# Plonky3/Plonky3-recursion

Measured on AMD Instinct MI355X. Metric: prove_next_layer ms + Poseidon2 perms/s, KoalaBear 2^20-row circuit, 1/8 GPU, lower is better.
Workload: dtype u32 Montgomery (31-bit prime field, degree-4 extension); Poseidon2 hashing as exact integers in f64; 1 GPU; prove_next_layer (verifier-circuit run on the device + prove_all_tables) of the synthetic koala-bear 2^20-row recursion layer: tables const/public/alu/poseidon2/recompose, FRI blowup 4, arity<=4, 54 queries, 15-bit PoW; circuit inputs + NextLayerPrepCache resident in HBM; field=koala-bear, log_height=20, independent_proofs=1, proof_bytes=612900, parallelism=1 independent proofs, one per GPU, no data-path collective

## Files before the change

### plonky3_recursion_amd/csrc/circuit_impl.hip.h

```cpp

#include "circuit_host.h"

namespace {

template <class PP, int D = 4>
__device__ __forceinline__ typename CircuitExt<PP, D>::type w_load(const uint32_t* __restrict__ w, uint32_t id) {
  typename CircuitExt<PP, D>::type e;
  if constexpr (D == 4) {
    const uint4 v = *reinterpret_cast<const uint4*>(w + (size_t)id * 4);
    e.c[0] = Fp<PP>::raw(v.x); e.c[1] = Fp<PP>::raw(v.y); e.c[2] = Fp<PP>::raw(v.z); e.c[3] = Fp<PP>::raw(v.w);
  } else {
#pragma unroll
    for (int k = 0; k < D; ++k) e.c[k] = Fp<PP>::raw(w[(size_t)id * D + k]);
  }
  return e;
}
template <class PP, int D = 4>
__device__ __forceinline__ void w_store(uint32_t* __restrict__ w, uint32_t id, const typename CircuitExt<PP, D>::type& e) {
  if constexpr (D == 4) {
    *reinterpret_cast<uint4*>(w + (size_t)id * 4) = make_uint4(e.c[0].v, e.c[1].v, e.c[2].v, e.c[3].v);
  } else {
#pragma unroll
    for (int k = 0; k < D; ++k) w[(size_t)id * D + k] = e.c[k].v;
  }
// ... 714 lines not shown
  atomicMin(&slot[v & 0x7FFFFFFFu], (uint32_t)k);
}
__global__ void __launch_bounds__(kBlock)
k_pd_check(const uint32_t* __restrict__ ids, size_t n, const uint32_t* __restrict__ row_of_id, size_t n_ids,
           const uint32_t* __restrict__ slot, uint32_t* __restrict__ err) {
  const size_t k = (size_t)blockIdx.x * kBlock + threadIdx.x;
  if (k >= n) return;
  const uint32_t id = ids[k];
  uint32_t code = 0;
  if (id >= n_ids || row_of_id[id] == kNoW) code = 1;
  else if (slot[row_of_id[id] & 0x7FFFFFFFu] != k) code = 2;
  else if (!(row_of_id[id] >> 31)) code = 3;
  if (code) atomicMin(err, ((uint32_t)k << 2) | code);
}

template <class PP>
std::unique_ptr<p3r_dinputs> circuit_inputs_upload(p3r_ctx* ctx, const p3r_circuit* C, const p3r_circuit_inputs* in) {
  if (C->n_public_rows && !in->public_values) fail(P3R_EINVAL, "PublicInputLengthMismatch: public_values is NULL");
  if (C->n_private_rows && !in->private_values) fail(P3R_EINVAL, "PrivateInputLengthMismatch: private_values is NULL");
  const size_t n_p2 = C->counts.n_p2, n_pd = in->n_private_data;
  if (n_pd && (!in->private_data_op_ids || !in->private_data_siblings)) fail(P3R_EINVAL, "private data arrays are NULL");
  auto D = std::make_unique<p3r_dinputs>();
  D->pub = upload_mont<PP>(ctx, in->public_values, C->n_public_rows * ctx->cfg.ext_degree, "public_values");
  D->priv = upload_mont<PP>(ctx, in->private_values, C->n_private_rows * ctx->cfg.ext_degree, "private_values");
  auto private_data = [&](size_t n_pd, const uint32_t* ids_host, const uint32_t* sib_host, size_t per_op, size_t n_rows,
                          const DevBuf& row_of_id, const DevBuf& other_row_of_id, DevBuf& sib, DevBuf& slot, const char* what) {
    sib = upload_mont<PP>(ctx, sib_host, n_pd * per_op, what);
    slot.alloc(std::max<size_t>(n_rows, 1));
    P3R_HIP(fill_async(ctx->stream, slot.p, 0xFF, std::max<size_t>(n_rows, 1) * 4));
    if (!n_pd) return;
    if (!row_of_id.p)
      fail(P3R_EINVAL, "NonPrimitiveOpIdOutOfRange { op_id: %u, max_ops: %zu } (%s)", ids_host[0], C->n_op_ids, what);
    DevBuf ids(n_pd), err(1);
    P3R_HIP(hipMemcpyAsync(ids.p, ids_host, n_pd * 4, hipMemcpyHostToDevice, ctx->stream));
    P3R_HIP(fill_async(ctx->stream, err.p, 0xFF, 4));
    hipLaunchKernelGGL(k_pd_claim, dim3(blocks_for(n_pd)), dim3(kBlock), 0, ctx->stream, ids.p, n_pd, row_of_id.p, C->n_op_ids, slot.p);
    hipLaunchKernelGGL(k_pd_check, dim3(blocks_for(n_pd)), dim3(kBlock), 0, ctx->stream, ids.p, n_pd, row_of_id.p, C->n_op_ids, slot.p, err.p);
    uint32_t e = 0;
    P3R_HIP(copy_sync(ctx->stream, &e, err.p, 4, hipMemcpyDeviceToHost));
    if (e != 0xFFFFFFFFu) {
      const uint32_t id = ids_host[e >> 2];
      switch (e & 3) {
        case 1: {
          uint32_t other = kNoW;
          if (other_row_of_id.p && id < C->n_op_ids) P3R_HIP(copy_sync(ctx->stream, &other, other_row_of_id.p + id, 4, hipMemcpyDeviceToHost));
          if (other != kNoW)
            fail(P3R_EINVAL, "IncorrectNonPrimitiveOpPrivateData: NonPrimitiveOpId(%u) is a permutation of the other width (%s)", id, what);
          fail(P3R_EINVAL, "NonPrimitiveOpIdOutOfRange { op_id: %u, max_ops: %zu }", id, C->n_op_ids);
        }
        case 2: fail(P3R_EINVAL, "IncorrectNonPrimitiveOpPrivateData: private data already set for NonPrimitiveOpId(%u)", id);
        default: fail(P3R_EINVAL, "IncorrectNonPrimitiveOpPrivateData: private data provided for non-Merkle operation NonPrimitiveOpId(%u)", id);
      }
    }
  };
  private_data(n_pd, in->private_data_op_ids, in->private_data_siblings, 8, n_p2, C->d_row_of_op_id, C->d_roww_of_op_id, D->sib, D->slot,
               "private_data_siblings");
  const size_t n_pdw = in->n_private_data_w32;
  if (n_pdw && (!in->private_data_w32_op_ids || !in->private_data_w32_siblings)) fail(P3R_EINVAL, "width-32 private data arrays are NULL");
  private_data(n_pdw, in->private_data_w32_op_ids, in->private_data_w32_siblings, 24, C->counts.n_p2w, C->d_roww_of_op_id, C->d_row_of_op_id,
               D->sib_w, D->slot_w, "private_data_w32_siblings");
  return D;
}

inline void run_raise_error(uint32_t e) {
  if (e != 0xFFFFFFFFu) {
    const uint32_t idx = e >> 3;
    if (idx == 0x1FFFFFFFu) fail(P3R_EINVAL, "WitnessConflict while applying witness_rewrite");
    fail(P3R_EINVAL, "%s at op %u", run_error_text(e & 7), idx);
  }
}

template <class PP>
std::unique_ptr<p3r_dtraces> circuit_run(p3r_ctx* ctx, const p3r_circuit* C, const p3r_dinputs* in,
                                         uint32_t* deferred_err = nullptr) {
  const RunSchedule& S = C->sched;
  const p3r_layer* L = C->layer.get();
  if (!S.deferred_error.empty()) fail(P3R_EINVAL, "%s", S.deferred_error.c_str());
  const size_t n_p2 = C->counts.n_p2;
// ... 79 lines not shown
    }
    dispatch_ext_degree<PP>((int)ext_d, [&](auto dc) {
    constexpr int DD = decltype(dc)::value;
    for (const auto& seg : S.segments) {
      if (seg.narrow) {
        hipLaunchKernelGGL((k_run_levels_narrow<PP, DD>), dim3(1), dim3(kNarrowBlock), 0, ctx->stream, A,
                           C->d_chunk_bounds.p + seg.chunk_begin, seg.n_chunks);
        continue;
      }
      const uint32_t l = seg.l0;
      const uint32_t nl = S.light_off[l + 1] - S.light_off[l], np = S.p2seg_off[l + 1] - S.p2seg_off[l];
      const uint32_t lb = (nl + kBlock - 1) / kBlock, pb = (np * 16 + kBlock - 1) / kBlock;
      const uint32_t nc = S.chain_off[l + 1] - S.chain_off[l], n_long = S.chain_long[l];
      const RunOp* steps = reinterpret_cast<const RunOp*>(C->d_chain_ops.p);
      const RunSchedule::ChainSeg* segs = reinterpret_cast<const RunSchedule::ChainSeg*>(C->d_chains.p) + S.chain_off[l];
      const uint32_t n_short = nc - n_long, cb = (n_short + kBlock / 64 - 1) / (kBlock / 64);
      const uint32_t npw = has_w32 ? S.p2wseg_off[l + 1] - S.p2wseg_off[l] : 0u, pwb = (npw * 32 + kBlock - 1) / kBlock;
      if (lb + pb + cb + pwb)
        hipLaunchKernelGGL((k_run_level<PP, DD>), dim3(pb + cb + lb + pwb), dim3(kBlock), 0, ctx->stream, A, S.p2seg_off[l], np, pb,
                           steps, segs + n_long, n_short, cb, S.light_off[l], nl, has_w32 ? S.p2wseg_off[l] : 0u, npw, pwb);
      if (n_long)
        hipLaunchKernelGGL((k_run_chains_block<PP, DD>), dim3(n_long), dim3(kLongChainBlock), 0, ctx->stream, A, steps, segs);
    }
    if (C->n_rewrite)
      hipLaunchKernelGGL((k_run_rewrite<PP, DD>), dim3(blocks_for(C->n_rewrite)), dim3(kBlock), 0, ctx->stream,
                         C->d_rewrite.p, C->n_rewrite, w.p, err.p);
    });
    if (cn.n_public)
      hipLaunchKernelGGL(k_run_gather<PP>, dim3(blocks_for(cn.n_public * ext_d)), dim3(kBlock), 0, ctx->stream,
                         C->d_public_out.p, cn.n_public, w.p, T->public_values.p, ext_d);
    P3R_HIP(hipGetLastError());
  }
  if (deferred_err) {
    P3R_HIP(hipMemcpyAsync(deferred_err, err.p, 4, hipMemcpyDeviceToHost, ctx->stream));
  } else {
    uint32_t e = 0;
    P3R_HIP(copy_sync(ctx->stream, &e, err.p, 4, hipMemcpyDeviceToHost));
    run_raise_error(e);
  }
  return T;
}

template <class PP>
void dtraces_get(p3r_ctx* ctx, const p3r_layer* L, const p3r_dtraces* t, uint32_t which, uint32_t* out, size_t out_len) {
  const auto& c = L->counts;
  auto plain_at = [&](const uint32_t* src, size_t n) {
    if (out_len != n) fail(P3R_EBUFFER, "array holds %zu values, caller asked for %zu", n, out_len);
    if (!n) return;
    DevBuf tmp(n);
    P3R_HIP(hipMemcpyAsync(tmp.p, src, n * 4, hipMemcpyDeviceToDevice, ctx->stream));
    hipLaunchKernelGGL(k_convert_inplace<PP>, dim3(blocks_for(n)), dim3(kBlock), 0, ctx->stream, tmp.p, n, 0);
    P3R_HIP(copy_sync(ctx->stream, out, tmp.p, n * 4, hipMemcpyDeviceToHost));
  };
  switch (which) {
    case P3R_TRACES_CONST_VALUES: plain_at(t->const_values.p, c.n_const * ctx->cfg.ext_degree); break;
    case P3R_TRACES_PUBLIC_VALUES: plain_at(t->public_values.p, c.n_public * ctx->cfg.ext_degree); break;
    case P3R_TRACES_ALU_VALUES: plain_at(t->alu_values.p, c.n_alu * 4 * ctx->cfg.ext_degree); break;
    case P3R_TRACES_RECOMPOSE_VALUES: plain_at(t->recompose_values.p, c.n_recompose * ctx->cfg.ext_degree); break;
    case P3R_TRACES_RECOMPOSE_COEFF_VALUES:
      plain_at(t->recompose_values.p + c.n_recompose * ctx->cfg.ext_degree, c.n_recompose_coeff * ctx->cfg.ext_degree);
      break;
    case P3R_TRACES_P2_INPUT_VALUES: {
      if (out_len != c.n_p2 * 16) fail(P3R_EBUFFER, "array holds %zu values, caller asked for %zu", c.n_p2 * 16, out_len);
      if (!c.n_p2) break;
      std::vector<uint32_t> full(t->p2->n * 16);
      download<PP>(ctx, t->p2->inputs.get(), full.data());
      std::copy(full.begin(), full.begin() + c.n_p2 * 16, out);
      break;
    }
    case P3R_TRACES_P2_FLAGS: {
// ... 45 lines not shown
```

### plonky3_recursion_amd/csrc/context.h

```cpp
#pragma once
#include <hip/hip_runtime.h>

#include <algorithm>
#include <array>
#include <atomic>
#include <cstdarg>
#include <cstdio>
#include <cstring>
#include <exception>
#include <functional>
#include <map>
#include <memory>
#include <chrono>
#include <mutex>
#include <stdexcept>
#include <string>
#include <thread>
#include <tuple>
#include <vector>

#include "../../include/p3r.h"
#include "error.h"
#include "field.h"
#include "poseidon2.h"
#include "proof_layout.h"
#include "mmcs4.h"

namespace p3r {

template <class Fn>
inline void host_parallel_for(size_t n, size_t min_chunk, Fn fn) {
  const size_t hw = std::max<size_t>(std::thread::hardware_concurrency(), 1);
  const size_t chunks = std::min<size_t>(std::min<size_t>(hw, 16), (n + min_chunk - 1) / std::max<size_t>(min_chunk, 1));
  if (chunks <= 1) { fn((size_t)0, n); return; }
  std::vector<std::exception_ptr> err(chunks);
  std::vector<std::thread> th;
  auto run = [&](size_t c) {
    try { fn(n * c / chunks, n * (c + 1) / chunks); } catch (...) { err[c] = std::current_exception(); }
  };
  for (size_t c = 1; c < chunks; ++c) th.emplace_back(run, c);
  run(0);
  for (auto& t : th) t.join();
  for (auto& e : err) if (e) std::rethrow_exception(e);
}

#define P3R_HIP(expr)                                                                   \
  do {                                                                                  \
    hipError_t e_ = (expr);                                                             \
    if (e_ != hipSuccess)                                                               \
      ::p3r::fail(e_ == hipErrorOutOfMemory ? P3R_ENOMEM : P3R_EHIP, "%s failed: %s",   \
                  #expr, hipGetErrorString(e_));                                        \
  } while (0)

struct DevPool;
struct PoolRegistry {
  std::mutex mu;
// ... 129 lines not shown
}
template <class T>
static __global__ void __launch_bounds__(256) k_copy_small(uint8_t* __restrict__ dst, const uint8_t* __restrict__ src, size_t n) {
  const size_t tid = (size_t)blockIdx.x * 256 + threadIdx.x, nt = (size_t)gridDim.x * 256;
  const size_t nq = n / sizeof(T);
  T* d = reinterpret_cast<T*>(dst);
  const T* q = reinterpret_cast<const T*>(src);
  for (size_t i = tid; i < nq; i += nt) d[i] = q[i];
  const size_t done = nq * sizeof(T);
  if (tid < n - done) dst[done + tid] = src[done + tid];
}
inline hipError_t fill_async(hipStream_t s, void* p, int byte, size_t bytes) {
  if (bytes == 0) return hipSuccess;
  host_mark("launch: fill");
  const uint32_t b = (uint32_t)byte & 0xFFu, pattern = b * 0x01010101u;
  const size_t blocks = std::min<size_t>((bytes / 16 + 255) / 256 + 1, 4096);
  hipLaunchKernelGGL(k_fill_bytes, dim3((unsigned)blocks), dim3(256), 0, s, static_cast<uint8_t*>(p), pattern, bytes);
  return hipGetLastError();
}
inline hipError_t copy_async_kernel(hipStream_t s, void* dst, const void* src, size_t bytes) {
  if (bytes == 0) return hipSuccess;
  host_mark("launch: copy");
  const uintptr_t both = reinterpret_cast<uintptr_t>(dst) | reinterpret_cast<uintptr_t>(src);
  const size_t w = (both & 15) == 0 ? 16 : (both & 3) == 0 ? 4 : 1;
  const size_t blocks = std::min<size_t>((bytes / w + 255) / 256 + 1, 4096);
  uint8_t* d = static_cast<uint8_t*>(dst);
  const uint8_t* q = static_cast<const uint8_t*>(src);
  if (w == 16) hipLaunchKernelGGL(k_copy_small<uint4>, dim3((unsigned)blocks), dim3(256), 0, s, d, q, bytes);
  else if (w == 4) hipLaunchKernelGGL(k_copy_small<uint32_t>, dim3((unsigned)blocks), dim3(256), 0, s, d, q, bytes);
  else hipLaunchKernelGGL(k_copy_small<uint8_t>, dim3((unsigned)blocks), dim3(256), 0, s, d, q, bytes);
  return hipGetLastError();
}

struct HostStage {
  static constexpr size_t kBytes = size_t(4) << 20;
  char* base = nullptr;
  char* base_dev = nullptr;
  size_t off = 0;
  HostStage() = default;
  HostStage(const HostStage&) = delete;
  HostStage& operator=(const HostStage&) = delete;
  ~HostStage() {
    if (base) (void)hipHostFree(base);
  }
  static constexpr size_t kWordBytes = 64;
  hipError_t ensure() {
    if (base) return hipSuccess;
    off = kWordBytes;
    hipError_t e = hipHostMalloc(reinterpret_cast<void**>(&base), kBytes, hipHostMallocMapped | hipHostMallocCoherent);
    if (e != hipSuccess) return e;
    return hipHostGetDevicePointer(reinterpret_cast<void**>(&base_dev), base, 0);
  }
  hipError_t words(uint32_t** out) {
    hipError_t e = ensure();
    *out = reinterpret_cast<uint32_t*>(base);
    return e;
  }
  hipError_t upload(hipStream_t s, void* dst, const void* src, size_t bytes) {
    if (bytes == 0) return hipSuccess;
    if (bytes > kBytes / 4) return copy_sync(s, dst, src, bytes, hipMemcpyHostToDevice);
    {
      hipError_t e = ensure();
      if (e != hipSuccess) return e;
    }
    const size_t need = (bytes + 63) & ~size_t(63);
    if (off + need > kBytes) {
      hipError_t e = hipStreamSynchronize(s);
      if (e != hipSuccess) return e;
      off = kWordBytes;
    }
    std::memcpy(base + off, src, bytes);
    hipError_t e = copy_async_kernel(s, dst, base_dev + off, bytes);
    off += need;
    return e;
  }
};

struct HostLanding {
  char* base = nullptr;
  size_t cap = 0;
  HostLanding() = default;
  HostLanding(const HostLanding&) = delete;
  HostLanding& operator=(const HostLanding&) = delete;
  ~HostLanding() {
    if (base) (void)hipHostFree(base);
  }
  hipError_t fetch(hipStream_t s, const void* dev, size_t bytes, const uint32_t** out) {
    if (bytes > cap) {
      if (base) (void)hipHostFree(base);
      base = nullptr;
      cap = 0;
      const size_t want = std::max(bytes * 2, size_t(1) << 20);
      hipError_t e = hipHostMalloc(reinterpret_cast<void**>(&base), want, hipHostMallocDefault);
      if (e != hipSuccess) return e;
      cap = want;
    }
    *out = reinterpret_cast<const uint32_t*>(base);
    if (bytes == 0) return hipStreamSynchronize(s);
    return copy_sync(s, base, dev, bytes, hipMemcpyDeviceToHost);
  }
};

static __global__ void __launch_bounds__(256) k_post_small(uint32_t* host_dst, const uint32_t* __restrict__ src, uint32_t n,
                                                    uint32_t* flag, uint32_t seq) {
  for (uint32_t i = threadIdx.x; i < n; i += 256) host_dst[i] = src[i];
  __threadfence_system();
  __syncthreads();
  if (threadIdx.x == 0) __hip_atomic_store(flag, seq, __ATOMIC_RELEASE, __HIP_MEMORY_SCOPE_SYSTEM);
}
struct HostPost {
  static constexpr size_t kWords = 16384;
  uint32_t* host = nullptr;
  uint32_t* dev = nullptr;
  uint32_t seq = 0;
  static constexpr int kSlots = 48;
  int slot = 0;
  bool in_proof = false;
  uint64_t shape = 0;
  int64_t expect_ns[kSlots] = {};
  void begin_proof(uint64_t shape_key) {
    slot = 0;
    in_proof = true;
    if (shape_key != shape) { shape = shape_key; std::fill(expect_ns, expect_ns + kSlots, 0); }
  }
  void end_proof() { in_proof = false; }
  HostPost() = default;
  HostPost(const HostPost&) = delete;
  HostPost& operator=(const HostPost&) = delete;
  ~HostPost() {
    if (host) (void)hipHostFree(host);
  }
  hipError_t post(hipStream_t s, const uint32_t* src, size_t words, const uint32_t** out) {
    if (!host) {
      hipError_t e = hipHostMalloc(reinterpret_cast<void**>(&host), (kWords + 16) * 4,
                                   hipHostMallocMapped | hipHostMallocCoherent);
      if (e != hipSuccess) return e;
      e = hipHostGetDevicePointer(reinterpret_cast<void**>(&dev), host, 0);
      if (e != hipSuccess) {
        (void)hipHostFree(host);
        host = nullptr;
        dev = nullptr;
        return e;
      }
      host[kWords] = 0;
    }
    *out = host;
    ++seq;
    hipLaunchKernelGGL(k_post_small, dim3(1), dim3(256), 0, s, dev, src, (uint32_t)words, dev + kWords, seq);
    hipError_t e = hipGetLastError();
    if (e != hipSuccess) return e;
    volatile uint32_t* flag = host + kWords;
    const int sl = slot < kSlots ? slot : kSlots - 1;
    if (in_proof) ++slot;
    const auto t0 = std::chrono::steady_clock::now();
    auto elapsed_ns = [&] { return (int64_t)std::chrono::duration_cast<std::chrono::nanoseconds>(std::chrono::steady_clock::now() - t0).count(); };
    const int64_t expect = in_proof ? expect_ns[sl] : 0;
    if (expect > 400000) {
      const int64_t until = expect - std::max<int64_t>(expect / 4, 200000);
      for (int64_t now = elapsed_ns(); now < until && *flag != seq; now = elapsed_ns())
        std::this_thread::sleep_for(std::chrono::nanoseconds(std::min<int64_t>(until - now, 500000)));
    }
    const int64_t awake_until = expect > 400000 ? expect + expect / 2 + 500000 : 0;
    for (uint64_t spins = 0;; ++spins) {
      if (*flag == seq) break;
      if (spins > (uint64_t(1) << 14) && (spins & 0x3F) == 0x3F) {
        if (awake_until && elapsed_ns() < awake_until) std::this_thread::yield();
        else if (spins > (uint64_t(1) << 17)) std::this_thread::sleep_for(std::chrono::microseconds(20));
        else std::this_thread::yield();
      }
      if ((spins & 0xFFF) == 0xFFF) {
        e = hipStreamQuery(s);
        if (e != hipErrorNotReady) {
          if (e != hipSuccess) return e;
          if (*flag == seq) break;
          return hipStreamSynchronize(s);
        }
      }
    }
    if (in_proof) expect_ns[sl] = elapsed_ns();
    std::atomic_thread_fence(std::memory_order_acquire);
    return hipSuccess;
  }
};

struct DevBuf {
  uint32_t* p = nullptr;
  size_t n = 0;
  std::shared_ptr<DevPool> pool;
  DevBuf() = default;
  explicit DevBuf(size_t cells) { alloc(cells); }
  DevBuf(const DevBuf&) = delete;
  DevBuf& operator=(const DevBuf&) = delete;
  DevBuf(DevBuf&& o) noexcept : p(o.p), n(o.n), pool(std::move(o.pool)) { o.p = nullptr; o.n = 0; }
  DevBuf& operator=(DevBuf&& o) noexcept {
    if (this != &o) { release(); p = o.p; n = o.n; pool = std::move(o.pool); o.p = nullptr; o.n = 0; }
    return *this;
  }
  ~DevBuf() { release(); }
  void alloc(size_t cells) {
    release();
    if (cells) {
      pool = tls_pool();
      if (!pool) fail(P3R_EINVAL, "device allocation outside a p3r API call");
      p = static_cast<uint32_t*>(pool->get(cells * sizeof(uint32_t)));
    }
    n = cells;
  }
  void release() {
    if (p) pool->put(p, n * sizeof(uint32_t));
    p = nullptr;
    n = 0;
    pool.reset();
  }
};
// ... 41 lines not shown
  const char* name;
  hipEvent_t a, b;
};
}

struct p3r_ctx {
  p3r_config cfg{};
  std::shared_ptr<p3r::DevPool> pool = std::make_shared<p3r::DevPool>();
  bool prof_enabled = false;
  std::vector<p3r::ProfRec> prof;
  std::vector<std::pair<std::string, double>> stage_ms;
  std::string cur_stage;
  double cur_stage_t0 = 0;
  int partial_rounds = 0;
  hipStream_t stream = nullptr;
  int n_cus = 256;
  p3r::DevBuf rc;
  p3r::DevBuf rc_f64;
  const double* rcd() const { return reinterpret_cast<const double*>(rc_f64.p); }
  size_t rcd_w32_at = 0;
  const double* rcd_w32() const { return rcd() + rcd_w32_at; }
  p3r::DevBuf p2_diag;
  std::vector<uint32_t> rc_canonical;
  std::vector<uint8_t> fri_log_arities;
  p3r::ProofLayout proof_layout;
  std::vector<uint32_t> rc_mont_host;
  std::string err;
  bool w32_diag_builtin = false;
  bool w32_unacknowledged = false;
  uint64_t zk_nonce = 0;
  uint32_t zk_key[8] = {0, 0, 0, 0, 0, 0, 0, 0};
  std::vector<uint8_t> pending_proof;
  p3r::HostStage stage;
  p3r::HostLanding landing;
  p3r::HostPost post;
  std::map<std::string, p3r::DevBuf> const_tables;

  struct NttTable { p3r::DevBuf lo, hi; };
  std::map<std::tuple<int, int, int, uint32_t>, NttTable> ntt_tables;
};

inline hipError_t fetch_small(p3r_ctx* ctx, const uint32_t* src, size_t words, uint32_t* dst) {
  if (words == 0) return hipSuccess;
  if (words <= p3r::HostPost::kWords) {
    const uint32_t* got = nullptr;
    p3r::host_mark("fetch: posted, waiting for the GPU");
    hipError_t e = ctx->post.post(ctx->stream, src, words, &got);
    p3r::host_mark("fetch: arrived");
    if (e != hipSuccess) return e;
    std::memcpy(dst, got, words * 4);
    return hipSuccess;
  }
  return p3r::copy_sync(ctx->stream, dst, src, words * 4, hipMemcpyDeviceToHost);
}
```

### plonky3_recursion_amd/csrc/mmcs_impl.hip.h

```cpp

namespace {

template <class PP>
void hash_rows(p3r_ctx* ctx, const std::vector<std::vector<const p3r_dmat*>>& classes,
               const std::vector<uint32_t*>& digs) {
  std::vector<HashRowsJob> jobs;
  for (size_t c = 0; c < classes.size(); ++c) {
    std::vector<const uint32_t*> cols;
    for (const p3r_dmat* m : classes[c])
      for (size_t k = 0; k < m->w; ++k) cols.push_back(m->d + k * m->h);
    HashRowsJob j{};
    j.cols = col_table(ctx, cols);
    j.dig = digs[c];
    j.h = classes[c][0]->h;
    j.wtot = (int)cols.size();
    jobs.push_back(j);
  }
  std::stable_sort(jobs.begin(), jobs.end(),
                   [](const HashRowsJob& a, const HashRowsJob& b) { return a.wtot > b.wtot; });
  uint32_t blocks = 0;
  double perms = 0;
  for (auto& j : jobs) {
    j.block0 = blocks;
    blocks += blocks_for(j.h);
// ... 253 lines not shown
  const size_t S = (size_t)tree->salt_elems, per = S ? 2 : 1, n_mats = tree->mats.size() / per;
  const size_t w_rows = tree->total_width, w_salts = n_mats * S, w_proof = mmcs_proof_len(tree->levels) * P2_DIGEST;
  const size_t words = w_rows + w_salts + w_proof;
  if (words >> 31 || n >> 31) fail(P3R_EUNSUPPORTED, "open_batch of %zu indices of %zu words each", n, words);
  std::vector<OpenItem> items;
  size_t off = 0;
  for (size_t i = 0; i < n_mats; ++i) {
    const p3r_dmat* m = tree->mats[i * per];
    const uint32_t shift = (uint32_t)(tree->log_max_h - log2_exact(m->h, "matrix height"));
    if (m->w) items.push_back(OpenItem{m->d, m->h, (uint32_t)off, shift, 0, 0});
    off += m->w;
    if (S) items.push_back(OpenItem{tree->mats[i * per + 1]->d, m->h, (uint32_t)(w_rows + i * S), shift, 0, 0});
  }
  off = w_rows + w_salts;
  const size_t last = (size_t(1) << tree->log_max_h) - 1;
  for (size_t l = 0; l < tree->levels.size(); ++l) {
    const MmcsLevel& lv = tree->levels[l];
    if (((last >> lv.bits) | (size_t)(lv.step - 1)) >= tree->layer_n[l]) fail(P3R_EHIP, "internal: Merkle layer %zu shorter than its level", l);
    for (int j = 0; j + 1 < lv.step; ++j, off += P2_DIGEST)
      items.push_back(OpenItem{tree->layers[l].p, tree->layer_n[l], (uint32_t)off, (uint32_t)lv.bits, (uint32_t)lv.step, (uint32_t)j});
  }
  if (!words) return;
  std::stable_sort(items.begin(), items.end(), [](const OpenItem& a, const OpenItem& b) { return a.dst < b.dst; });
  DevBuf d_items((items.size() * sizeof(OpenItem) + 3) / 4), d_idx(n), d_out(n * words);
  P3R_HIP(ctx->stage.upload(ctx->stream, d_items.p, items.data(), items.size() * sizeof(OpenItem)));
  P3R_HIP(ctx->stage.upload(ctx->stream, d_idx.p, idx32.data(), n * 4));
  {
    ProfScope ps(ctx, "mmcs_open_batch");
    hipLaunchKernelGGL(k_mmcs_open_batch<PP>, dim3((unsigned)n), dim3(256), 0, ctx->stream,
                       reinterpret_cast<const OpenItem*>(d_items.p), (uint32_t)items.size(), d_idx.p, (uint32_t)words, d_out.p);
    P3R_HIP(hipGetLastError());
  }
  const uint32_t* got = nullptr;
  P3R_HIP(ctx->landing.fetch(ctx->stream, d_out.p, n * words * 4, &got));
  for (size_t i = 0; i < n; ++i) {
    const uint32_t* g = got + i * words;
    std::memcpy(opened + i * w_rows, g, w_rows * 4);
    if (w_salts) std::memcpy(salts + i * w_salts, g + w_rows, w_salts * 4);
    std::memcpy(proofs + i * w_proof, g + w_rows + w_salts, w_proof * 4);
  }
}

}
```

### plonky3_recursion_amd/csrc/open_impl.hip.h

```cpp
#pragma once
#include <array>
#include <map>
#include <optional>

#include "tu_api.h"
#include "profile.h"

namespace p3r {

template <class PP, int DC>
struct OpenPlan {
  using F = Fp<PP>;
  using E = typename Chal<PP, DC>::type;
  p3r_ctx* ctx;
  std::vector<DevBuf> keep;
  std::vector<OpenWeightJob<DC>> wjobs;
  std::vector<OpenJob> djobs;
  std::map<std::array<uint64_t, 6>, const uint32_t*> wcache;
  uint32_t wblocks = 0, dblocks = 0;
  uint64_t used = 0;

  explicit OpenPlan(p3r_ctx* c) : ctx(c) {}

  const uint32_t* weights(size_t n, int log_n, const E& u, bool bit_reversed) {
// ... 52 lines not shown

  void launch(const char* weights_name, const char* dot_name, const char* reduce_name, void (*dot)(const OpenJob*, int),
              void (*reduce)(const OpenJob*, int, uint64_t, uint32_t*), uint32_t* out) {
    auto upload_jobs = [&](const auto& v) {
      using T = typename std::decay_t<decltype(v)>::value_type;
      keep.emplace_back((v.size() * sizeof(T) + 3) / 4);
      P3R_HIP(ctx->stage.upload(ctx->stream, keep.back().p, v.data(), v.size() * sizeof(T)));
      return reinterpret_cast<const T*>(keep.back().p);
    };
    const OpenWeightJob<DC>* d_w = upload_jobs(wjobs);
    const OpenJob* d_j = upload_jobs(djobs);
    std::optional<ProfScope> ps;
    ps.emplace(ctx, weights_name);
    hipLaunchKernelGGL((k_bary_weights<PP, DC>), dim3(wblocks), dim3(kBlock), 0, ctx->stream, d_w, (int)wjobs.size());
    ps.emplace(ctx, dot_name);
    hipLaunchKernelGGL(dot, dim3(dblocks), dim3(kBlock), 0, ctx->stream, d_j, (int)djobs.size());
    if (reduce_name) ps.emplace(ctx, reduce_name);
    hipLaunchKernelGGL(reduce, dim3((unsigned)((used + kBlock - 1) / kBlock)), dim3(kBlock), 0, ctx->stream, d_j, (int)djobs.size(),
                       used, out);
    ps.reset();
    P3R_HIP(hipGetLastError());
  }
};

template <class PP, int DC = 4>
struct Opener {
  using F = Fp<PP>;
  using E = typename Chal<PP, DC>::type;
  p3r_ctx* ctx;
  OpenPlan<PP, DC> plan;
  struct Job { size_t off; int P, w; };
  std::vector<Job> jobs;
  DevBuf out;

  explicit Opener(p3r_ctx* c) : ctx(c), plan(c) {}

  size_t open(const uint32_t* mat, size_t n, int w, F dshift, const std::vector<E>& points) {
    const int P = (int)points.size(), log_n = log2_exact(n, "trace height");
    const F inv_shift = dshift.inv();
    const uint32_t* wt[2];
    for (int p = 0; p < P; ++p) wt[p] = plan.weights(n, log_n, points[p] * inv_shift, false);
    const uint64_t out0 = plan.add_pass(mat, n, n, 1, w, wt, P, pts_cols(P), 2 * kBlock);
    jobs.push_back({(size_t)(out0 / DC), P, w});
    return jobs.size() - 1;
  }

  const uint32_t* values_dev(size_t job, int point) const {
    return out.p + (jobs[job].off + (size_t)point * jobs[job].w) * DC;
  }

  std::vector<std::vector<std::vector<E>>> finish() {
    if (jobs.empty()) return {};
    const size_t words = (size_t)plan.used;
    out.alloc(words);
    plan.launch("open_weights", "open_dot", nullptr, k_open_dot<PP, DC>, k_open_reduce<PP, DC, false>, out.p);
    const uint32_t* raw = nullptr;
    if (words <= HostPost::kWords) P3R_HIP(ctx->post.post(ctx->stream, out.p, words, &raw));
    else P3R_HIP(ctx->landing.fetch(ctx->stream, out.p, words * 4, &raw));
    plan.keep.clear();
    std::vector<std::vector<std::vector<E>>> res(jobs.size());
    for (size_t j = 0; j < jobs.size(); ++j) {
      res[j].resize(jobs[j].P);
      for (int p = 0; p < jobs[j].P; ++p) {
        res[j][p].resize(jobs[j].w);
        for (int c = 0; c < jobs[j].w; ++c)
          for (int k = 0; k < DC; ++k)
            res[j][p][c].c[k] = F::raw(raw[(jobs[j].off + (size_t)p * jobs[j].w + c) * DC + k]);
      }
    }
    return res;
  }
};

}
```

### plonky3_recursion_amd/csrc/p3r_core.hip

```cpp
#include "context.h"
#include "kernels.hip.h"
#include "kernels_stark.hip.h"
#include "kernels_coop.hip.h"
#include "tu_api.h"
#include "air_program.h"
#include "profile.h"
#include "run_schedule.h"
#include "prep_device.h"
#include "host_abi.h"

#include <sys/random.h>

#include <algorithm>
#include <cerrno>
#include <future>
#include <numeric>
#include <unordered_map>

using namespace p3r;

namespace {

thread_local std::string g_create_error;

// ... 1092 lines not shown
}
int p3r_circuit_prepared_on_device(const p3r_circuit* circuit) { return circuit && circuit->prepared_on_device ? 1 : 0; }
p3r_dinputs* p3r_circuit_inputs_upload(p3r_ctx* ctx, const p3r_circuit* circuit, const p3r_circuit_inputs* inputs) {
  p3r_dinputs* out = nullptr;
  guard(ctx, [&] {
    if (!circuit || !inputs) fail(P3R_EINVAL, "NULL argument");
    out = P3R_FIELD_CALL(ctx, circuit_inputs_upload, ctx, circuit, inputs).release();
  });
  return out;
}
void p3r_circuit_inputs_free(p3r_ctx* ctx, p3r_dinputs* inputs) {
  if (ctx) (void)hipStreamSynchronize(ctx->stream);
  delete inputs;
}
p3r_dtraces* p3r_circuit_run_resident(p3r_ctx* ctx, const p3r_circuit* circuit, const p3r_dinputs* inputs) {
  p3r_dtraces* out = nullptr;
  guard(ctx, [&] {
    if (!circuit || !inputs) fail(P3R_EINVAL, "NULL argument");
    out = P3R_FIELD_CALL(ctx, circuit_run, ctx, circuit, inputs).release();
  });
  return out;
}
p3r_dtraces* p3r_circuit_run(p3r_ctx* ctx, const p3r_circuit* circuit, const p3r_circuit_inputs* inputs) {
  p3r_dtraces* out = nullptr;
  guard(ctx, [&] {
    if (!circuit || !inputs) fail(P3R_EINVAL, "NULL argument");
    auto d = P3R_FIELD_CALL(ctx, circuit_inputs_upload, ctx, circuit, inputs);
    out = P3R_FIELD_CALL(ctx, circuit_run, ctx, circuit, d.get()).release();
  });
  return out;
}
static void prove_next_layer_impl(p3r_ctx* ctx, const p3r_circuit* circuit, const p3r_dinputs* d, uint32_t flags,
                                  uint8_t* proof_buf, size_t proof_cap, size_t* proof_len) {
  uint32_t* run_err = nullptr;
  P3R_HIP(ctx->stage.words(&run_err));
  *run_err = 0xFFFFFFFFu;
  auto t = P3R_FIELD_CALL(ctx, circuit_run, ctx, circuit, d, run_err);
  std::vector<uint8_t> bytes;
  try {
    bytes = P3R_FIELD_CALL(ctx, prove_all_tables, ctx, circuit->layer.get(), t.get(),
                           (flags & P3R_PROVE_CANONICAL_FIELD_ENCODING) != 0);
  } catch (...) {
    if (hipStreamSynchronize(ctx->stream) == hipSuccess) run_raise_error(*run_err);
    throw;
  }
  run_raise_error(*run_err);
  emit_proof(ctx, std::move(bytes), proof_buf, proof_cap, proof_len);
}
int p3r_prove_next_layer(p3r_ctx* ctx, const p3r_circuit* circuit, const p3r_circuit_inputs* inputs,
                         uint32_t flags, uint8_t* proof_buf, size_t proof_cap, size_t* proof_len) {
  return guard(ctx, [&] {
    if (!circuit || !inputs || !proof_len || (!proof_buf && proof_cap)) fail(P3R_EINVAL, "bad arguments");
    auto d = P3R_FIELD_CALL(ctx, circuit_inputs_upload, ctx, circuit, inputs);
    prove_next_layer_impl(ctx, circuit, d.get(), flags, proof_buf, proof_cap, proof_len);
  });
}
int p3r_prove_next_layer_resident(p3r_ctx* ctx, const p3r_circuit* circuit, const p3r_dinputs* inputs,
                                  uint32_t flags, uint8_t* proof_buf, size_t proof_cap, size_t* proof_len) {
  return guard(ctx, [&] {
    if (!circuit || !inputs || !proof_len || (!proof_buf && proof_cap)) fail(P3R_EINVAL, "bad arguments");
    prove_next_layer_impl(ctx, circuit, inputs, flags, proof_buf, proof_cap, proof_len);
  });
}
int p3r_dtraces_get(p3r_ctx* ctx, const p3r_layer* layer, const p3r_dtraces* traces, uint32_t which,
                    uint32_t* out, size_t out_len) {
  return guard(ctx, [&] {
    if (!layer || !traces || (!out && out_len)) fail(P3R_EINVAL, "NULL argument");
    P3R_FIELD_CALL(ctx, dtraces_get, ctx, layer, traces, which, out, out_len);
  });
}
// ... 42 lines not shown
```

### plonky3_recursion_amd/csrc/prove_impl.hip.h

```cpp
#include "host_transcript.h"
#include "kernels_stark.hip.h"
#include "kernels_fri_reduce.hip.h"
#include "kernels_zk.hip.h"
#include "open_impl.hip.h"

struct p3r_prep {
  std::vector<p3r::AirParams> airs;
  std::vector<std::unique_ptr<p3r_dmat>> traces;
  std::vector<std::unique_ptr<p3r_dmat>> evals;
  std::vector<std::unique_ptr<p3r_dmat>> ldes;
  std::vector<size_t> heights;
  int zk_codewords = -1;
  const p3r_dmat* committed(size_t i) const { return evals.empty() ? traces[i].get() : evals[i].get(); }
  std::unique_ptr<p3r_tree> tree;
  std::vector<uint32_t> cap_canonical;
};

namespace {

template <class PP, int DC = 4>
EW<DC> to_e4(const typename Chal<PP, DC>::type& e) { return e4_store<PP, DC>(e); }

template <class PP, int DC = 4>
std::vector<typename Chal<PP, DC>::type> download_ef(p3r_ctx* ctx, const uint32_t* dev, size_t count) {
// ... 564 lines not shown
      auto m = dmat_alloc(2 * n, (size_t)DC + R);
      ZkChunkJob j{};
      j.q = quot_round.mats[k].ev->d; j.q_odd = q_odd[k]->d; j.t_odd = t_odd[k]->d; j.dst = m->d;
      j.n = n; j.log_n = log_n[quot_round.mats[k].inst]; j.DC = DC; j.R = R;
      j.stream = zk_stream_id(ZK_ROUND_QUOTIENT, k);
      j.block0 = (uint32_t)blocks;
      blocks += (uint64_t)(DC + R) * ((2 * n + kBlock - 1) / kBlock);
      jobs.push_back(j);
      quot_round.mats[k].ev = m.get();
      quot_round.keep.push_back(std::move(m));
    }
    if (blocks >= (uint64_t(1) << 31)) fail(P3R_EUNSUPPORTED, "ZK chunk launch of %llu tiles", (unsigned long long)blocks);
    DevBuf d_jobs((jobs.size() * sizeof(ZkChunkJob) + 3) / 4);
    P3R_HIP(ctx->stage.upload(ctx->stream, d_jobs.p, jobs.data(), jobs.size() * sizeof(ZkChunkJob)));
    {
      ProfScope ps(ctx, "zk_chunks");
      hipLaunchKernelGGL(k_zk_chunk<PP>, dim3((unsigned)blocks), dim3(kBlock), 0, ctx->stream,
                         reinterpret_cast<const ZkChunkJob*>(d_jobs.p), (int)jobs.size(), zk_key);
    }
    P3R_HIP(hipGetLastError());
    for (auto& m : q_odd) quot_round.keep.push_back(std::move(m));
    for (auto& m : t_odd) quot_round.keep.push_back(std::move(m));
  }

  void openings() {
    prof_stage(ctx, "openings");
    for (Round* r : rounds())
      for (Mat& m : r->mats) {
        m.z = {zeta};
        if (r == &prep_round || r == &perm_round || (r == &main_round && air_uses_next(prep->airs[m.inst])))
          m.z.push_back(zeta * F::two_adic_generator(log_n[m.inst]));
        m.job = op.open(m.ev->d, m.ev->h, (int)m.ev->w, m.shift, m.z);
      }
    auto all = op.finish();
    launch_inv_points();
    for (Round* r : rounds())
      for (Mat& m : r->mats)
        for (auto& pv : all[m.job]) {
          for (auto& v : pv) ch.observe_ext(v);
          m.vals.emplace_back(pv.begin(), pv.end() - R);
          m.codewords.emplace_back(pv.end() - R, pv.end());
        }
    check_at_zeta();
  }

  static std::array<uint64_t, 6> inv_key(int lh, const E& z) {
    std::array<uint64_t, 6> key{(uint64_t)lh, 0, 0, 0, 0, 0};
    for (int k = 0; k < DC; ++k) key[1 + k] = z.c[k].v;
    return key;
  }

  void launch_inv_points() {
    std::vector<FriInvJobT<DC>> inv_jobs;
    uint32_t inv_blocks = 0;
    for (Round* r : rounds())
      for (const Mat& m : r->mats) {
        const int lh = log_e[m.inst] + log_blowup;
        for (const E& z : m.z) {
          const auto key = inv_key(lh, z);
          if (inv_cache.count(key)) continue;
          inv_keep.emplace_back((size_t)DC << lh);
          FriInvJobT<DC> j{};
          j.inv = inv_keep.back().p;
          j.h = uint64_t(1) << lh;
          j.log_h = lh;
          if (lh < 2) fail(P3R_EINVAL, "FRI: an LDE of fewer than four rows");
          j.w_h = F::two_adic_generator(lh).v;
          j.w_4 = F::two_adic_generator(2).v;
          j.z = to_e4<PP, DC>(z);
          j.block0 = inv_blocks;
          inv_blocks += blocks_for((size_t(1) << lh) / 4);
          inv_jobs.push_back(j);
          inv_cache.emplace(key, j.inv);
        }
      }
    inv_keep.emplace_back((inv_jobs.size() * sizeof(FriInvJobT<DC>) + 3) / 4);
// ... 255 lines not shown
      QRound qr;
      for (const p3r_dmat* m : t->mats) {
        const int lh = log2_exact(m->h, "height");
        qr.rows.emplace_back(push(m->d, m->h, (uint32_t)m->w, (uint32_t)(log_max - lh), 0, 1), (uint32_t)m->w);
      }
      qr.tree_shift = tree_shift;
      qr.path = push_path(t, tree_shift);
      qrounds.push_back(std::move(qr));
    }
    int shift = 0;
    for (auto& ph : phases) {
      const size_t arity = size_t(1) << ph.la, n_in = ph.rows << ph.la;
      QPhase qp;
      qp.shift = shift;
      for (size_t j = 0; j < arity; ++j)
        qp.sib_at[j] = push(ph.folded_in.p + j, n_in, DC, (uint32_t)(shift + ph.la), 0, (uint32_t)arity);
      if (ph.tree->salt_elems)
        qp.salt_at = push(ph.tree->phase_salts.p, n_in, (uint32_t)ph.tree->salt_elems, (uint32_t)(shift + ph.la), 0, (uint32_t)arity);
      qp.path = push_path(ph.tree.get(), (uint32_t)(shift + ph.la));
      qphases.push_back(std::move(qp));
      shift += ph.la;
    }
    words_per_query = cursor;
    const auto* d_items = static_cast<const QueryItem*>(const_table(ctx, q_items.data(), q_items.size() * sizeof(QueryItem)));
    std::vector<uint32_t> idx32(indices.begin(), indices.end());
    DevBuf d_idx(idx32.size()), d_out((size_t)words_per_query * indices.size());
    hipError_t e = ctx->stage.upload(ctx->stream, d_idx.p, idx32.data(), idx32.size() * 4);
    if (e == hipSuccess) {
      ProfScope ps(ctx, "query_gather");
      hipLaunchKernelGGL(k_gather<PP>, dim3((unsigned)q_items.size(), (unsigned)indices.size()), dim3(64), 0, ctx->stream,
                         d_items, d_idx.p, words_per_query, d_out.p);
      e = hipGetLastError();
    }
    if (e == hipSuccess) e = ctx->landing.fetch(ctx->stream, d_out.p, d_out.n * 4, &gathered);
    P3R_HIP(e);
  }

  void write_path(const QPath& qp, const uint32_t* g, size_t tree_index) {
    W.varint(mmcs_proof_len(qp.t->levels));
    const uint32_t* sibs = g + qp.at;
    const std::vector<MmcsLevel>& lv = qp.t->levels;
    for (size_t l = 0; l < lv.size();) {
      size_t run = 0;
      while (l + run < lv.size() && lv[l + run].step == 2) ++run;
      W.words(sibs, run * P2_DIGEST);
      sibs += run * P2_DIGEST;
      l += run;
      if (l == lv.size()) break;
      const size_t step = lv[l].step, pos = (tree_index >> lv[l].bits) & (step - 1);
      for (size_t j = 0; j < step; ++j)
        if (j != pos) W.words(sibs + ((j ^ pos) - 1) * P2_DIGEST, P2_DIGEST);
      sibs += (step - 1) * P2_DIGEST;
      ++l;
    }
  }

  void write_queries() {
    W.varint(indices.size());
    for (size_t qi = 0; qi < indices.size(); ++qi) {
      const uint32_t* g = gathered + (size_t)qi * words_per_query;
      W.varint(qrounds.size());
      for (auto& qr : qrounds) {
        const size_t step = qr.path.t->salt_elems ? 2 : 1;
        for (size_t first = 0; first < step; ++first) {
          W.varint(qr.rows.size() / step);
          for (size_t k = first; k < qr.rows.size(); k += step) {
            W.varint(qr.rows[k].second);
// ... 91 lines not shown
            if (layouts[i].n_groups) { W.byte(1); W.ef(terminals[i]); } else W.byte(0);
          break;
        default:
          W.varint(ni);
          for (size_t i = 0; i < ni; ++i) W.varint(log_e[i]);
          break;
      }
    }
  }
};

template <class PP, int DC = 4>
std::vector<uint8_t> prove_batch(p3r_ctx* ctx, const p3r_prep* prep, const p3r_dmat* const* mains, size_t ni,
                                 bool canonical_encoding) {
  host_timeline_begin();
  {
    uint64_t shape = 0x9E3779B97F4A7C15ull ^ ni;
    for (size_t i = 0; i < ni; ++i) shape = (shape ^ (mains[i]->h * 31 + mains[i]->w)) * 0x100000001B3ull;
    if (ctx->prof_enabled) ctx->post.end_proof(); else ctx->post.begin_proof(shape);
  }
  struct EndProofWaits {
    HostPost& p;
    ~EndProofWaits() { p.end_proof(); }
  } end_proof_waits{ctx->post};
  if (ni != prep->airs.size()) fail(P3R_EINVAL, "%zu traces for %zu preprocessed instances", ni, prep->airs.size());
  if (prep->zk_codewords != zk_codewords(ctx->cfg)) fail(P3R_EINVAL, "the preprocessed data was committed under another ZK setting");
  BatchProver<PP, DC> pf(ctx, prep, mains, ni, canonical_encoding);
  pf.main_lde_commit();
  pf.transcript_head();
  pf.logup_aux_commit();
  pf.quotient_commit();
  pf.openings();
  pf.fri_reduce();
  pf.fri_commit_phase();
  pf.queries();
  pf.serialize();
  P3R_HIP(hipStreamSynchronize(ctx->stream));
  prof_stage(ctx, nullptr);
  host_timeline_dump();
  return pf.W.take();
}

template <class PP>
std::vector<uint8_t> prove_batch_any(p3r_ctx* ctx, const p3r_prep* prep, const p3r_dmat* const* mains, size_t ni,
                                     bool canonical_encoding) {
  if (ctx->cfg.challenge_degree == 5) {
    if constexpr (kHasQuintic<PP>) return prove_batch<PP, 5>(ctx, prep, mains, ni, canonical_encoding);
    else fail(P3R_EUNSUPPORTED, "UnsupportedChallengeDegree: the quintic challenge field is KoalaBear's");
  }
  return prove_batch<PP, 4>(ctx, prep, mains, ni, canonical_encoding);
}

}
```

Before: 26.71 ms.

## Route device-to-host readbacks through mapped landing buffers and overlap opening fetch

Replaces hipMemcpy/copy_sync device-to-host readbacks with a kernel that writes directly into mapped coherent host memory, followed by a flag post that the host polls. The opening readback is split into launch and collect so the inverse-point launch runs before the host waits, and the check_at_zeta step moves after fri_reduce. Small uploads and error fetches also go through the staged and mapped path. This is meant to cut synchronous memcpy latency and host stalls, at the cost of more complex ordering and a spin-wait on a host flag.

```diff
diff --git a/plonky3_recursion_amd/csrc/circuit_impl.hip.h b/plonky3_recursion_amd/csrc/circuit_impl.hip.h
--- a/plonky3_recursion_amd/csrc/circuit_impl.hip.h
+++ b/plonky3_recursion_amd/csrc/circuit_impl.hip.h
@@ -770,18 +770,18 @@
     if (!row_of_id.p)
       fail(P3R_EINVAL, "NonPrimitiveOpIdOutOfRange { op_id: %u, max_ops: %zu } (%s)", ids_host[0], C->n_op_ids, what);
     DevBuf ids(n_pd), err(1);
-    P3R_HIP(hipMemcpyAsync(ids.p, ids_host, n_pd * 4, hipMemcpyHostToDevice, ctx->stream));
+    P3R_HIP(ctx->stage.upload(ctx->stream, ids.p, ids_host, n_pd * 4));
     P3R_HIP(fill_async(ctx->stream, err.p, 0xFF, 4));
     hipLaunchKernelGGL(k_pd_claim, dim3(blocks_for(n_pd)), dim3(kBlock), 0, ctx->stream, ids.p, n_pd, row_of_id.p, C->n_op_ids, slot.p);
     hipLaunchKernelGGL(k_pd_check, dim3(blocks_for(n_pd)), dim3(kBlock), 0, ctx->stream, ids.p, n_pd, row_of_id.p, C->n_op_ids, slot.p, err.p);
     uint32_t e = 0;
-    P3R_HIP(copy_sync(ctx->stream, &e, err.p, 4, hipMemcpyDeviceToHost));
+    P3R_HIP(fetch_small(ctx, err.p, 1, &e));
     if (e != 0xFFFFFFFFu) {
       const uint32_t id = ids_host[e >> 2];
       switch (e & 3) {
         case 1: {
           uint32_t other = kNoW;
-          if (other_row_of_id.p && id < C->n_op_ids) P3R_HIP(copy_sync(ctx->stream, &other, other_row_of_id.p + id, 4, hipMemcpyDeviceToHost));
+          if (other_row_of_id.p && id < C->n_op_ids) P3R_HIP(fetch_small(ctx, other_row_of_id.p + id, 1, &other));
           if (other != kNoW)
             fail(P3R_EINVAL, "IncorrectNonPrimitiveOpPrivateData: NonPrimitiveOpId(%u) is a permutation of the other width (%s)", id, what);
           fail(P3R_EINVAL, "NonPrimitiveOpIdOutOfRange { op_id: %u, max_ops: %zu }", id, C->n_op_ids);
@@ -927,10 +927,10 @@
     P3R_HIP(hipGetLastError());
   }
   if (deferred_err) {
-    P3R_HIP(hipMemcpyAsync(deferred_err, err.p, 4, hipMemcpyDeviceToHost, ctx->stream));
+    P3R_HIP(copy_to_host_kernel(ctx->stream, deferred_err, err.p, 4));
   } else {
     uint32_t e = 0;
-    P3R_HIP(copy_sync(ctx->stream, &e, err.p, 4, hipMemcpyDeviceToHost));
+    P3R_HIP(fetch_small(ctx, err.p, 1, &e));
     run_raise_error(e);
   }
   return T;
diff --git a/plonky3_recursion_amd/csrc/context.h b/plonky3_recursion_amd/csrc/context.h
--- a/plonky3_recursion_amd/csrc/context.h
+++ b/plonky3_recursion_amd/csrc/context.h
@@ -22,6 +22,7 @@
 #include "../../include/p3r.h"
 #include "error.h"
 #include "field.h"
+#include "host_buffers.h"
 #include "poseidon2.h"
 #include "proof_layout.h"
 #include "mmcs4.h"
@@ -217,6 +218,37 @@
   return hipGetLastError();
 }
 
+template <class T>
+static __global__ void __launch_bounds__(256) k_copy_to_host(uint8_t* dst, const uint8_t* __restrict__ src, size_t n) {
+  const size_t tid = (size_t)blockIdx.x * 256 + threadIdx.x, nt = (size_t)gridDim.x * 256;
+  const size_t nq = n / sizeof(T);
+  T* d = reinterpret_cast<T*>(dst);
+  const T* q = reinterpret_cast<const T*>(src);
+  for (size_t i = tid; i < nq; i += nt) d[i] = q[i];
+  const size_t done = nq * sizeof(T);
+  if (tid < n - done) dst[done + tid] = src[done + tid];
+  __threadfence_system();
+}
+inline hipError_t copy_to_host_kernel(hipStream_t s, void* host_dev, const void* src, size_t bytes) {
+  if (bytes == 0) return hipSuccess;
+  host_mark("launch: copy to host");
+  const uintptr_t both = reinterpret_cast<uintptr_t>(host_dev) | reinterpret_cast<uintptr_t>(src);
+  const size_t w = (both & 15) == 0 ? 16 : (both & 3) == 0 ? 4 : 1;
+  const size_t blocks = std::min<size_t>((bytes / w + 255) / 256 + 1, 4096);
+  uint8_t* d = static_cast<uint8_t*>(host_dev);
+  const uint8_t* q = static_cast<const uint8_t*>(src);
+  if (w == 16) hipLaunchKernelGGL(k_copy_to_host<uint4>, dim3((unsigned)blocks), dim3(256), 0, s, d, q, bytes);
+  else if (w == 4) hipLaunchKernelGGL(k_copy_to_host<uint32_t>, dim3((unsigned)blocks), dim3(256), 0, s, d, q, bytes);
+  else hipLaunchKernelGGL(k_copy_to_host<uint8_t>, dim3((unsigned)blocks), dim3(256), 0, s, d, q, bytes);
+  return hipGetLastError();
+}
+
+struct HipMappedOps {
+  int alloc(void** host, size_t bytes) { return (int)hipHostMalloc(host, bytes, hipHostMallocMapped | hipHostMallocCoherent); }
+  int map(void** dev, void* host) { return (int)hipHostGetDevicePointer(dev, host, 0); }
+  void release(void* host) { (void)hipHostFree(host); }
+};
+
 struct HostStage {
   static constexpr size_t kBytes = size_t(4) << 20;
   char* base = nullptr;
@@ -231,14 +263,19 @@
   static constexpr size_t kWordBytes = 64;
   hipError_t ensure() {
     if (base) return hipSuccess;
+    MappedPair m;
+    HipMappedOps ops;
+    hipError_t e = (hipError_t)mapped_reserve(ops, m, kBytes, kBytes);
+    if (e != hipSuccess) return e;
+    base = m.host;
+    base_dev = m.dev;
     off = kWordBytes;
-    hipError_t e = hipHostMalloc(reinterpret_cast<void**>(&base), kBytes, hipHostMallocMapped | hipHostMallocCoherent);
-    if (e != hipSuccess) return e;
-    return hipHostGetDevicePointer(reinterpret_cast<void**>(&base_dev), base, 0);
-  }
-  hipError_t words(uint32_t** out) {
+    return hipSuccess;
+  }
+  hipError_t words(uint32_t** out, uint32_t** out_dev) {
     hipError_t e = ensure();
     *out = reinterpret_cast<uint32_t*>(base);
+    *out_dev = reinterpret_cast<uint32_t*>(base_dev);
     return e;
   }
   hipError_t upload(hipStream_t s, void* dst, const void* src, size_t bytes) {
@@ -248,41 +285,15 @@
       hipError_t e = ensure();
       if (e != hipSuccess) return e;
     }
-    const size_t need = (bytes + 63) & ~size_t(63);
-    if (off + need > kBytes) {
+    const RingSlot slot = ring_place(off, bytes, kBytes, kWordBytes);
+    if (slot.wrap) {
       hipError_t e = hipStreamSynchronize(s);
       if (e != hipSuccess) return e;
-      off = kWordBytes;
-    }
-    std::memcpy(base + off, src, bytes);
-    hipError_t e = copy_async_kernel(s, dst, base_dev + off, bytes);
-    off += need;
+    }
+    std::memcpy(base + slot.at, src, bytes);
+    hipError_t e = copy_async_kernel(s, dst, base_dev + slot.at, bytes);
+    off = slot.next;
     return e;
-  }
-};
-
-struct HostLanding {
-  char* base = nullptr;
-  size_t cap = 0;
-  HostLanding() = default;
-  HostLanding(const HostLanding&) = delete;
-  HostLanding& operator=(const HostLanding&) = delete;
-  ~HostLanding() {
-    if (base) (void)hipHostFree(base);
-  }
-  hipError_t fetch(hipStream_t s, const void* dev, size_t bytes, const uint32_t** out) {
-    if (bytes > cap) {
-      if (base) (void)hipHostFree(base);
-      base = nullptr;
-      cap = 0;
-      const size_t want = std::max(bytes * 2, size_t(1) << 20);
-      hipError_t e = hipHostMalloc(reinterpret_cast<void**>(&base), want, hipHostMallocDefault);
-      if (e != hipSuccess) return e;
-      cap = want;
-    }
-    *out = reinterpret_cast<const uint32_t*>(base);
-    if (bytes == 0) return hipStreamSynchronize(s);
-    return copy_sync(s, base, dev, bytes, hipMemcpyDeviceToHost);
   }
 };
 
@@ -316,24 +327,27 @@
     if (host) (void)hipHostFree(host);
   }
   hipError_t post(hipStream_t s, const uint32_t* src, size_t words, const uint32_t** out) {
+    hipError_t e = launch(s, src, words, out);
+    if (e != hipSuccess) return e;
+    return wait(s);
+  }
+  hipError_t launch(hipStream_t s, const uint32_t* src, size_t words, const uint32_t** out) {
     if (!host) {
-      hipError_t e = hipHostMalloc(reinterpret_cast<void**>(&host), (kWords + 16) * 4,
-                                   hipHostMallocMapped | hipHostMallocCoherent);
+      MappedPair m;
+      HipMappedOps ops;
+      hipError_t e = (hipError_t)mapped_reserve(ops, m, (kWords + 16) * 4, (kWords + 16) * 4);
       if (e != hipSuccess) return e;
-      e = hipHostGetDevicePointer(reinterpret_cast<void**>(&dev), host, 0);
-      if (e != hipSuccess) {
-        (void)hipHostFree(host);
-        host = nullptr;
-        dev = nullptr;
-        return e;
-      }
+      host = reinterpret_cast<uint32_t*>(m.host);
+      dev = reinterpret_cast<uint32_t*>(m.dev);
       host[kWords] = 0;
     }
     *out = host;
     ++seq;
     hipLaunchKernelGGL(k_post_small, dim3(1), dim3(256), 0, s, dev, src, (uint32_t)words, dev + kWords, seq);
-    hipError_t e = hipGetLastError();
-    if (e != hipSuccess) return e;
+    return hipGetLastError();
+  }
+  hipError_t wait(hipStream_t s) {
+    hipError_t e = hipSuccess;
     volatile uint32_t* flag = host + kWords;
     const int sl = slot < kSlots ? slot : kSlots - 1;
     if (in_proof) ++slot;
@@ -365,6 +379,31 @@
     if (in_proof) expect_ns[sl] = elapsed_ns();
     std::atomic_thread_fence(std::memory_order_acquire);
     return hipSuccess;
+  }
+};
+
+struct HostLanding {
+  MappedPair m;
+  HostLanding() = default;
+  HostLanding(const HostLanding&) = delete;
+  HostLanding& operator=(const HostLanding&) = delete;
+  ~HostLanding() {
+    if (m.host) (void)hipHostFree(m.host);
+  }
+  hipError_t launch(hipStream_t s, HostPost& post, const void* dev, size_t bytes, const uint32_t** out) {
+    HipMappedOps ops;
+    hipError_t e = (hipError_t)mapped_reserve(ops, m, bytes, landing_capacity(bytes));
+    if (e != hipSuccess) return e;
+    *out = reinterpret_cast<const uint32_t*>(m.host);
+    e = copy_to_host_kernel(s, m.dev, dev, bytes);
+    if (e != hipSuccess) return e;
+    const uint32_t* unused = nullptr;
+    return post.launch(s, nullptr, 0, &unused);
+  }
+  hipError_t fetch(hipStream_t s, HostPost& post, const void* dev, size_t bytes, const uint32_t** out) {
+    hipError_t e = launch(s, post, dev, bytes, out);
+    if (e != hipSuccess) return e;
+    return post.wait(s);
   }
 };
 
@@ -472,8 +511,8 @@
   uint32_t zk_key[8] = {0, 0, 0, 0, 0, 0, 0, 0};
   std::vector<uint8_t> pending_proof;
   p3r::HostStage stage;
+  p3r::HostPost post;
   p3r::HostLanding landing;
-  p3r::HostPost post;
   std::map<std::string, p3r::DevBuf> const_tables;
 
   struct NttTable { p3r::DevBuf lo, hi; };
@@ -491,5 +530,11 @@
     std::memcpy(dst, got, words * 4);
     return hipSuccess;
   }
-  return p3r::copy_sync(ctx->stream, dst, src, words * 4, hipMemcpyDeviceToHost);
-}
+  const uint32_t* got = nullptr;
+  p3r::host_mark("fetch: landing, waiting for the GPU");
+  hipError_t e = ctx->landing.fetch(ctx->stream, ctx->post, src, words * 4, &got);
+  p3r::host_mark("fetch: arrived");
+  if (e != hipSuccess) return e;
+  std::memcpy(dst, got, words * 4);
+  return hipSuccess;
+}
diff --git a/plonky3_recursion_amd/csrc/host_buffers.h b/plonky3_recursion_amd/csrc/host_buffers.h
--- /dev/null
+++ b/plonky3_recursion_amd/csrc/host_buffers.h
@@ -0,0 +1,45 @@
+#pragma once
+#include <algorithm>
+#include <cstddef>
+
+namespace p3r {
+
+struct RingSlot {
+  size_t at, next;
+  bool wrap;
+};
+inline RingSlot ring_place(size_t off, size_t bytes, size_t cap, size_t head) {
+  const size_t need = (bytes + 63) & ~size_t(63);
+  const bool wrap = off + need > cap;
+  const size_t at = wrap ? head : off;
+  return {at, at + need, wrap};
+}
+
+inline size_t landing_capacity(size_t bytes) { return std::max(bytes * 2, size_t(1) << 20); }
+
+struct MappedPair {
+  char* host = nullptr;
+  char* dev = nullptr;
+  size_t cap = 0;
+};
+template <class Ops>
+int mapped_reserve(Ops& ops, MappedPair& m, size_t bytes, size_t want) {
+  if (bytes <= m.cap) return 0;
+  if (m.host) ops.release(m.host);
+  m = MappedPair{};
+  void* h = nullptr;
+  int e = ops.alloc(&h, want);
+  if (e != 0) return e;
+  void* d = nullptr;
+  e = ops.map(&d, h);
+  if (e != 0) {
+    ops.release(h);
+    return e;
+  }
+  m.host = static_cast<char*>(h);
+  m.dev = static_cast<char*>(d);
+  m.cap = want;
+  return 0;
+}
+
+}
diff --git a/plonky3_recursion_amd/csrc/mmcs_impl.hip.h b/plonky3_recursion_amd/csrc/mmcs_impl.hip.h
--- a/plonky3_recursion_amd/csrc/mmcs_impl.hip.h
+++ b/plonky3_recursion_amd/csrc/mmcs_impl.hip.h
@@ -309,7 +309,7 @@
     P3R_HIP(hipGetLastError());
   }
   const uint32_t* got = nullptr;
-  P3R_HIP(ctx->landing.fetch(ctx->stream, d_out.p, n * words * 4, &got));
+  P3R_HIP(ctx->landing.fetch(ctx->stream, ctx->post, d_out.p, n * words * 4, &got));
   for (size_t i = 0; i < n; ++i) {
     const uint32_t* g = got + i * words;
     std::memcpy(opened + i * w_rows, g, w_rows * 4);
diff --git a/plonky3_recursion_amd/csrc/open_impl.hip.h b/plonky3_recursion_amd/csrc/open_impl.hip.h
--- a/plonky3_recursion_amd/csrc/open_impl.hip.h
+++ b/plonky3_recursion_amd/csrc/open_impl.hip.h
@@ -108,6 +108,7 @@
   struct Job { size_t off; int P, w; };
   std::vector<Job> jobs;
   DevBuf out;
+  const uint32_t* raw = nullptr;
 
   explicit Opener(p3r_ctx* c) : ctx(c), plan(c) {}
 
@@ -126,13 +127,22 @@
   }
 
   std::vector<std::vector<std::vector<E>>> finish() {
-    if (jobs.empty()) return {};
+    launch();
+    return collect();
+  }
+
+  void launch() {
+    if (jobs.empty()) return;
     const size_t words = (size_t)plan.used;
     out.alloc(words);
     plan.launch("open_weights", "open_dot", nullptr, k_open_dot<PP, DC>, k_open_reduce<PP, DC, false>, out.p);
-    const uint32_t* raw = nullptr;
-    if (words <= HostPost::kWords) P3R_HIP(ctx->post.post(ctx->stream, out.p, words, &raw));
-    else P3R_HIP(ctx->landing.fetch(ctx->stream, out.p, words * 4, &raw));
+    if (words <= HostPost::kWords) P3R_HIP(ctx->post.launch(ctx->stream, out.p, words, &raw));
+    else P3R_HIP(ctx->landing.launch(ctx->stream, ctx->post, out.p, words * 4, &raw));
+  }
+
+  std::vector<std::vector<std::vector<E>>> collect() {
+    if (jobs.empty()) return {};
+    P3R_HIP(ctx->post.wait(ctx->stream));
     plan.keep.clear();
     std::vector<std::vector<std::vector<E>>> res(jobs.size());
     for (size_t j = 0; j < jobs.size(); ++j) {
diff --git a/plonky3_recursion_amd/csrc/p3r_core.hip b/plonky3_recursion_amd/csrc/p3r_core.hip
--- a/plonky3_recursion_amd/csrc/p3r_core.hip
+++ b/plonky3_recursion_amd/csrc/p3r_core.hip
@@ -1148,10 +1148,10 @@
 }
 static void prove_next_layer_impl(p3r_ctx* ctx, const p3r_circuit* circuit, const p3r_dinputs* d, uint32_t flags,
                                   uint8_t* proof_buf, size_t proof_cap, size_t* proof_len) {
-  uint32_t* run_err = nullptr;
-  P3R_HIP(ctx->stage.words(&run_err));
+  uint32_t *run_err = nullptr, *run_err_dev = nullptr;
+  P3R_HIP(ctx->stage.words(&run_err, &run_err_dev));
   *run_err = 0xFFFFFFFFu;
-  auto t = P3R_FIELD_CALL(ctx, circuit_run, ctx, circuit, d, run_err);
+  auto t = P3R_FIELD_CALL(ctx, circuit_run, ctx, circuit, d, run_err_dev);
   std::vector<uint8_t> bytes;
   try {
     bytes = P3R_FIELD_CALL(ctx, prove_all_tables, ctx, circuit->layer.get(), t.get(),
diff --git a/plonky3_recursion_amd/csrc/prove_impl.hip.h b/plonky3_recursion_amd/csrc/prove_impl.hip.h
--- a/plonky3_recursion_amd/csrc/prove_impl.hip.h
+++ b/plonky3_recursion_amd/csrc/prove_impl.hip.h
@@ -620,8 +620,9 @@
           m.z.push_back(zeta * F::two_adic_generator(log_n[m.inst]));
         m.job = op.open(m.ev->d, m.ev->h, (int)m.ev->w, m.shift, m.z);
       }
-    auto all = op.finish();
+    op.launch();
     launch_inv_points();
+    auto all = op.collect();
     for (Round* r : rounds())
       for (Mat& m : r->mats)
         for (auto& pv : all[m.job]) {
@@ -629,7 +630,6 @@
           m.vals.emplace_back(pv.begin(), pv.end() - R);
           m.codewords.emplace_back(pv.end() - R, pv.end());
         }
-    check_at_zeta();
   }
 
   static std::array<uint64_t, 6> inv_key(int lh, const E& z) {
@@ -951,7 +951,7 @@
                          d_items, d_idx.p, words_per_query, d_out.p);
       e = hipGetLastError();
     }
-    if (e == hipSuccess) e = ctx->landing.fetch(ctx->stream, d_out.p, d_out.n * 4, &gathered);
+    if (e == hipSuccess) e = ctx->landing.fetch(ctx->stream, ctx->post, d_out.p, d_out.n * 4, &gathered);
     P3R_HIP(e);
   }
 
@@ -1109,6 +1109,7 @@
   pf.quotient_commit();
   pf.openings();
   pf.fri_reduce();
+  pf.check_at_zeta();
   pf.fri_commit_phase();
   pf.queries();
   pf.serialize();
```

Measured after the change: 26.49 ms (median of 5 runs). Within noise of the previous version (-0.8%).
